# MarineRoboticsGroup/mac

Measured on AMD Instinct MI355X. Metric: frank_wolfe_iters_per_sec, higher is better.
Workload: dtype f64; 1 GPU; configs[3]: ER N=100000 ~2M candidates, chain fixed, K=10%; N=100000, m_candidates=2001737, K=200173, fixed_edges=99999, fw_iters=209, parallelism=single GPU

## Files before the change

### mac_amd/_lib.py

```python
from __future__ import annotations

import ctypes as C
import os

import numpy as np

_HERE = os.path.dirname(os.path.abspath(__file__))
LIB_PATH = os.environ.get("MACHIP_LIB") or os.path.join(_HERE, "libmachip.so")

OK, NOT_CONVERGED, DISCONNECTED, BAD_ARG, HIP_ERROR, RCCL_ERROR, NO_DEVICE = range(7)
STATUS_NAMES = ["OK", "NOT_CONVERGED", "DISCONNECTED", "BAD_ARG", "HIP_ERROR", "RCCL_ERROR", "NO_DEVICE"]


class MachipError(RuntimeError):
    def __init__(self, status, msg):
        super().__init__(f"libmachip: {STATUS_NAMES[status] if 0 <= status < 7 else status}: {msg}")
        self.status = status


class NotConverged(MachipError):
    pass


class Disconnected(MachipError):
# ... 68 lines not shown
    "machip_synchronize": (C.c_int, [C.c_void_p]),
    "machip_membench": (C.c_int, [C.c_int, C.c_int64, C.c_int, _f64p, _f64p]),
    "machip_host_tridiag_smallest": (C.c_int, [_f64p, _f64p, C.c_int, _f64p, _f64p]),
    "machip_host_follow_records": (C.c_int, [_f64p, C.c_int, C.c_int, C.c_double, C.c_double, C.c_int, C.POINTER(C.c_int), C.c_int,
                                             C.POINTER(C.c_int), C.POINTER(C.c_int), C.POINTER(C.c_double)]),
    "machip_release_cache": (None, []),
    "machip_panel_plan": (C.c_int, [C.c_int64, C.c_int64, C.c_int, C.POINTER(C.c_int)]),
    "machip_esp_create": (C.c_int, [C.c_int, C.c_int64, C.c_int64, _i32p, _i32p, _f64p, C.c_int64, _i32p, _i32p, _f64p,
                                    C.c_int, C.c_int, C.POINTER(C.c_void_p)]),
    "machip_esp_destroy": (None, [C.c_void_p]),
    "machip_esp_select": (C.c_int, [C.c_void_p, C.c_int, C.POINTER(C.c_int64), _i32p, _f64p, _f64p]),
    "machip_esp_weighted_resistances": (C.c_int, [C.c_void_p, _f64p]),
    "machip_esp_info": (C.c_int, [C.c_void_p, _i32p, C.POINTER(C.c_double)]),
    "machip_esp_tree_plan": (C.c_int, [C.c_int64, C.c_int64, _i32p, _i32p, _f64p, _i32p, _f64p, _i32p, _i32p, C.POINTER(C.c_int64),
                                       _i32p, _i32p, _f64p]),
    "machip_esp_seeds": (C.c_int, [C.c_void_p, C.POINTER(C.c_int64)]),
    "machip_esp_relax_eval": (C.c_int, [C.c_void_p, _f64p, C.POINTER(C.c_double), _f64p]),
    "machip_esp_relax_run": (C.c_int, [C.c_void_p, C.c_int64, C.c_int, C.c_double, C.c_double, _f64p, _f64p, _f64p, _f64p,
                                       C.POINTER(C.c_int), C.POINTER(C.c_double)]),
    "machip_esp_relax_inner": (C.c_int, [C.c_void_p, _f64p, _f64p, C.POINTER(C.c_double)]),
    "machip_esp_relax_info": (C.c_int, [C.c_void_p, _i32p]),
    "machip_esp_relax_gram": (C.c_int, [C.c_void_p, _f64p, C.c_int64]),
    "machip_esp_exchange": (C.c_int, [C.c_void_p, C.c_int64, _i32p, C.c_int64, C.c_double, _i32p, _i32p, _i32p, _f64p,
                                      C.POINTER(C.c_int64), C.POINTER(C.c_int32), _f64p]),
    "machip_eig_create": (C.c_int, [C.c_int, C.c_int64, C.c_int64, _i32p, _i32p, _f64p, C.c_int64, _i32p, _i32p, _f64p,
                                    C.c_int, C.c_int, C.c_int, C.POINTER(C.c_void_p)]),
    "machip_eig_destroy": (None, [C.c_void_p]),
    "machip_eig_select": (C.c_int, [C.c_void_p, C.c_int64, _i32p, _f64p, _f64p]),
    "machip_eig_candidate_lambda2": (C.c_int, [C.c_void_p, _f64p]),
    "machip_eig_candidate_bounds": (C.c_int, [C.c_void_p, _f64p]),
    "machip_eig_info": (C.c_int, [C.c_void_p, _i32p, _f64p, C.c_int64, _i32p, _i32p]),
}


def load():
    global _lib
    if _lib is not None:
        return _lib
    if not os.path.exists(LIB_PATH):
        raise ImportError(f"{LIB_PATH} is missing: build it with `python __graft_entry__.py` "
                          "(hipcc --offload-arch=gfx950); mac_amd has no CPU fallback")
    lib = C.CDLL(LIB_PATH, mode=C.RTLD_GLOBAL)
    for name, (res, args) in SIGNATURES.items():
        fn = getattr(lib, name)
        fn.restype = res
        fn.argtypes = args
    _lib = lib
    import atexit
    atexit.register(lib.machip_release_cache)
    return lib


OPTION_AUTO = -(1 << 63)
CREATION_OPTIONS = frozenset({"asm_g", "asm_maxgrid", "vbudget_mb", "vcap"})


def option_names():
    lib, out, i = load(), [], 0
    while True:
        nm = lib.machip_option_name(i)
        if nm is None:
            return out
        out.append(nm.decode())
        i += 1


def set_default_option(name, value=None):
    check(load().machip_set_option(None, name.encode(), OPTION_AUTO if value is None else int(value)))


class default_options:

    def __init__(self, **opts):
        self.opts = opts

    def __enter__(self):
        lib = load()
        self.old = {}
        for k, v in self.opts.items():
            cur = C.c_int64(0)
            check(lib.machip_get_option(None, k.encode(), C.byref(cur)))
            self.old[k] = cur.value
            set_default_option(k, v)
        return self

    def __exit__(self, *exc):
        for k, v in self.old.items():
            check(load().machip_set_option(None, k.encode(), v))
        return False


def membench(nbytes=1 << 30, reps=10, device=0):
    r, t = C.c_double(0.0), C.c_double(0.0)
    check(load().machip_membench(int(device), int(nbytes), int(reps), C.byref(r), C.byref(t)))
    return r.value, t.value


def device_count():
    return int(load().machip_device_count())


def require_device():
    n = device_count()
    if n <= 0:
        raise MachipError(NO_DEVICE, "no MI355X / HIP device visible; mac_amd has no CPU fallback")
    return n

# ... 512 lines not shown
```

### mac_amd/csrc/kernels.h

```cpp
#pragma once
#include "common.h"

namespace machip {

template <typename T>
struct CsrViewT {
    int n;
    const int* rowptr;
    const int* col;
    const T* val;
};
using CsrView = CsrViewT<double>;

struct PatternView {
    int n;
    const int* prow;
    const int* pcol;
    const int* pk;
    const double* pw;
};

struct LanState {
    int jA;
    int jB;
    int epoch;
    int jN;
};

struct LanView {
    int n;
    LanState* st;
    double* u;
    double* w;
    double* V;
    double* alpha;
    double* beta;
    double* l1;
    double* part_u;
    int P_u;
    double* part_a;
    int P_a;
};

constexpr int kAsmGrid = 4096;
__global__ __launch_bounds__(kBlock) void k_x_bits(const double* __restrict__ x, long m, double tol, unsigned long long* __restrict__ bits) {
    for (long i = (long)blockIdx.x * kBlock + threadIdx.x; i < m; i += (long)gridDim.x * kBlock) {
        const unsigned long long bal = __ballot(x[i] > tol);
        if ((threadIdx.x & 63) == 0) bits[i >> 6] = bal;
    }
}
__device__ __forceinline__ bool x_bit(const unsigned int* __restrict__ bits32, int k) { return (bits32[k >> 5] >> (k & 31)) & 1u; }

template <int G>
__global__ __launch_bounds__(kBlock) void k_asm_count(PatternView P, const unsigned int* __restrict__ xbits,
                                                      int rows_per_block,
                                                      int* __restrict__ cnt, int* __restrict__ blk_sum,
                                                      int* __restrict__ hsum = nullptr) {
    __shared__ int sm[4];
    constexpr int GPB = kBlock / G;
    const int lane = threadIdx.x % G, g = threadIdx.x / G;
    const int r0 = blockIdx.x * rows_per_block;
    const int r1 = min(P.n, r0 + rows_per_block);
    int local = 0, supp = 0, mx = 0;
    for (int r = r0 + g; r < r1; r += GPB) {
        const int b = P.prow[r], e = P.prow[r + 1];
        int c = 0, sc = 0;
        for (int p = b + lane; p < e; p += G) {
            const int k = P.pk[p];
            const bool cand = k >= 0;
            const bool act = cand ? x_bit(xbits, k) : true;
            c += act;
            sc += (cand && act);
        }
        c = group_sum_i<G>(c);
        sc = group_sum_i<G>(sc);
        if (lane == 0) {
            cnt[r] = c + 1;
            local += c + 1;
            supp += sc;
            mx = max(mx, c + 1);
        }
    }
    const int tot = block_sum_i(local, sm);
    const int stot = block_sum_i(supp, sm);
#pragma unroll
    for (int o = 32; o > 0; o >>= 1) mx = max(mx, __shfl_xor(mx, o, kWave));
    __syncthreads();
    if ((threadIdx.x & 63) == 0) sm[threadIdx.x >> 6] = mx;
    __syncthreads();
    if (threadIdx.x == 0) {
        blk_sum[blockIdx.x] = tot;
        blk_sum[kAsmGrid + blockIdx.x] = stot;
        const int longest = max(max(sm[0], sm[1]), max(sm[2], sm[3]));
        blk_sum[2 * kAsmGrid + blockIdx.x] = longest;
        if (hsum) {
            hsum[blockIdx.x] = tot; hsum[kAsmGrid + blockIdx.x] = stot; hsum[2 * kAsmGrid + blockIdx.x] = longest;
        }
    }
}

struct PanSpec {
    int NP = 0;
    int C = 1;
    int band = 0;
    int* ps = nullptr;
    double* bd = nullptr;
    int* bpk = nullptr;
    int* ovf = nullptr;
};

template <int G>
__global__ __launch_bounds__(kBlock) void k_asm_fill(PatternView P, const unsigned int* __restrict__ xbits, const double* __restrict__ x,
                                                     int rows_per_block,
                                                     const int* __restrict__ cnt,
                                                     const int* __restrict__ blk_sum,
                                                     int* __restrict__ rowptr, int* __restrict__ col,
                                                     double* __restrict__ val,
                                                     double* __restrict__ blk_lnorm, PanSpec S = PanSpec()) {
    extern __shared__ __attribute__((aligned(16))) char smem_raw[];
    int* s_off = reinterpret_cast<int*>(smem_raw);
    __shared__ int sm_i[4];
    __shared__ double sm_d[4];
    __shared__ int s_chunk[kBlock];
    constexpr int GPB = kBlock / G;
    const int tid = threadIdx.x;
    const int lane = tid % G, g = tid / G;
    const int r0 = blockIdx.x * rows_per_block;
    const int r1 = min(P.n, r0 + rows_per_block);
    const int nr = max(0, r1 - r0);

    int acc = 0;
    for (int b = tid; b < (int)blockIdx.x; b += kBlock) acc += blk_sum[b];
    const int base = block_sum_i(acc, sm_i);

    const int per = (nr + kBlock - 1) / kBlock;
    int csum = 0;
    for (int i = 0; i < per; ++i) {
        const int idx = tid * per + i;
        if (idx < nr) csum += cnt[r0 + idx];
    }
    {
        const int ln = tid & 63, wv = tid >> 6;
        int x = csum;
        for (int o = 1; o < 64; o <<= 1) { const int y = __shfl_up(x, o, kWave); if (ln >= o) x += y; }
        if (ln == 63) s_chunk[wv] = x;
        __syncthreads();
        int before = 0;
        for (int q = 0; q < wv; ++q) before += s_chunk[q];
        int run = before + x - csum;
        if (tid == kBlock - 1) s_off[nr] = before + x;
        for (int i = 0; i < per; ++i) {
            const int idx = tid * per + i;
            if (idx < nr) { s_off[idx] = run; run += cnt[r0 + idx]; }
        }
    }
    __syncthreads();

    double lmax = 0.0;
    for (int r = r0 + g; r < r1; r += GPB) {
        const int b = P.prow[r], e = P.prow[r + 1];
        const int out = base + s_off[r - r0];
        int pos = out + 1;
        double dsum = 0.0, asum = 0.0;
        int lastpid = 0;
        int hb = 0x7fffffff, hn = 0;
        double vl = 0.0, vu = 0.0;
        const int gbase = ((tid & 63) / G) * G;
        for (int p0 = b; p0 < e; p0 += G) {
            const int p = p0 + lane;
            const bool in = p < e;
            const int kc = in ? P.pk[p] : -1;
            const double wgt = in ? P.pw[p] : 0.0;
            const double xk = kc >= 0 ? x[kc] : 1.0;
            const bool act = in && (kc < 0 || x_bit(xbits, kc));
            const double v = act ? xk * wgt : 0.0;
            const unsigned long long bal = __ballot(act);
            unsigned long long gm;
            if (G == 64) gm = bal;
            else gm = (bal >> gbase) & ((1ull << (G & 63)) - 1ull);
            const unsigned long long below = gm & ((1ull << lane) - 1ull);
            const int before = __popcll(below);
            const int c = act ? P.pcol[p] : 0;
            if (act) { col[pos + before] = c; val[pos + before] = -v; }
            if (S.NP) {
                const int pid = act ? c / S.C : 0;
                const int src = below ? 63 - __builtin_clzll(below) : 0;
                const int got = __shfl(pid, gbase + src, kWave);
                const int ppid = below ? got : lastpid;
                if (act) {
                    const int q = pos + before;
                    for (int pp = ppid + 1; pp <= pid; ++pp) S.ps[(size_t)r * (S.NP + 1) + pp] = q;
                    if (S.band && (c == r - 1 || c == r + 1)) {
                        hb = min(hb, q); hn += 1;
                        if (c == r - 1) vl += -v; else vu += -v;
                    }
                }
                if (gm) lastpid = __shfl(pid, gbase + 63 - __builtin_clzll(gm), kWave);
            }
            pos += __popcll(gm);
            dsum += v;
            asum += fabs(v);
        }
        dsum = group_sum<G>(dsum);
        asum = group_sum<G>(asum);
        if (S.NP) {
            if (lane == 0) S.ps[(size_t)r * (S.NP + 1)] = out + 1;
            for (int pp = lastpid + 1 + lane; pp <= S.NP; pp += G) S.ps[(size_t)r * (S.NP + 1) + pp] = pos;
            if (S.band) {
                hn = group_sum_i<G>(hn);
                vl = group_sum<G>(vl); vu = group_sum<G>(vu);
#pragma unroll
                for (int o = G / 2; o > 0; o >>= 1) hb = min(hb, __shfl_xor(hb, o, kWave));
                if (lane == 0) {
                    S.bpk[r] = ((hn ? hb : pos) << 3) | min(hn, 7);
                    if (hn > 7) *S.ovf = 1;
                    S.bd[r] = dsum; S.bd[(size_t)P.n + r] = vl; S.bd[2 * (size_t)P.n + r] = vu;
                }
            }
        }
        if (lane == 0) {
            rowptr[r] = out;
            col[out] = r;
            val[out] = dsum;
            lmax = fmax(lmax, fabs(dsum) + asum);
        }
    }
    lmax = block_max(lmax, sm_d);
    if (tid == 0) {
        blk_lnorm[blockIdx.x] = lmax;
        if (blockIdx.x == gridDim.x - 1) rowptr[P.n] = base + s_off[nr];
    }
}

template <int G, class Op>
__device__ __forceinline__ void spmv_rows_vec(const CsrView& A, const double* __restrict__ x, Op& op) {
    constexpr int GPB = kBlock / G;
    const int lane = threadIdx.x % G, g = threadIdx.x / G;
    const int stride = gridDim.x * GPB;
    for (int r = blockIdx.x * GPB + g; r < A.n; r += 2 * stride) {
        const int r2 = r + stride;
        const bool two = r2 < A.n;
        const int b = A.rowptr[r], e = A.rowptr[r + 1];
        const int b2 = two ? A.rowptr[r2] : 0, e2 = two ? A.rowptr[r2 + 1] : 0;
        double acc = 0.0, acc2 = 0.0;
        int p = b + lane, q = b2 + lane;
        while (p < e || q < e2) {
            double v1 = 0.0, x1 = 0.0, v2 = 0.0, x2 = 0.0;
            if (p < e) { v1 = A.val[p]; x1 = op.gather(x, A.col[p]); }
            if (q < e2) { v2 = A.val[q]; x2 = op.gather(x, A.col[q]); }
            if (p < e) acc += v1 * x1;
            if (q < e2) acc2 += v2 * x2;
            p += G; q += G;
        }
        acc = group_sum<G>(acc);
        acc2 = group_sum<G>(acc2);
        if (lane == 0) { op.row(r, acc); if (two) op.row(r2, acc2); }
    }
}

constexpr int kStreamTile = 2048;

template <int TPR, class Op>
__device__ __forceinline__ void spmv_rows_stream(const CsrView& A, const double* __restrict__ x, Op& op,
                                                 double* prod, int* sptr) {
    constexpr int R = kBlock / TPR;
    const int tid = threadIdx.x;
    const int row = tid / TPR, sub = tid % TPR;
    for (int tile = blockIdx.x; tile * R < A.n; tile += gridDim.x) {
        const int r0 = tile * R;
        const int nr = min(R, A.n - r0);
        for (int i = tid; i <= nr; i += kBlock) sptr[i] = A.rowptr[r0 + i];
        __syncthreads();
        const int p0 = sptr[0], p1 = sptr[nr];
        double acc = 0.0;
        for (int base = p0; base < p1; base += kStreamTile) {
            const int cnt = min(kStreamTile, p1 - base);
            for (int i = tid; i < cnt; i += kBlock) prod[i] = A.val[base + i] * op.gather(x, A.col[base + i]);
            __syncthreads();
// ... 1130 lines not shown
```

### mac_amd/csrc/machip.hip

```cpp
#include <rccl/rccl.h>
#include <unistd.h>

#include <algorithm>
#include <atomic>
#include <cmath>
#include <chrono>
#include <condition_variable>
#include <functional>
#include <future>
#include <memory>
#include <mutex>
#include <numeric>
#include <thread>
#include <vector>

#include "solver.h"
#include "esp.h"
#include "esp_free.h"
#include "esp_tree.h"
#include "esp_relax.h"
#include "esp_exchange.h"
#include "eig.h"

namespace machip {
// ... 12 lines not shown
    auto state = std::make_shared<std::promise<int>>();
    std::future<int> fut = state->get_future();
    std::thread([state, fn] { int r = MACHIP_HIP_ERROR; try { r = fn(); } catch (...) {} state->set_value(r); }).detach();
    if (fut.wait_for(std::chrono::duration<double>(limit_s)) != std::future_status::ready)
        return fail(MACHIP_RCCL_ERROR, what + " did not return within " + std::to_string((int)limit_s) + " s (a peer rank is missing, or the fabric / bootstrap interface is not reachable; MACHIP_RCCL_TIMEOUT_S raises the limit)");
    return fut.get();
}
static double rccl_timeout_s() { const Options& opt = default_options(); const int t = OPT(rccl_timeout_s, 600); return t > 0 ? (double)t : 600.0; }

struct machip_problem;
struct LocalGroup {
    int nranks = 0;
    std::vector<double*> g;
    std::vector<machip_problem*> members;
    ShardGroup sg;
    bool shard_eig = false;
    int lead_status = MACHIP_OK;
    double lead_lam = 0.0;
    machip_solve_stats lead_stats{};
    std::string lead_err;
    ~LocalGroup() {
        for (ShardRank& r : sg.rk) for (hipEvent_t e : r.ev) if (e) (void)hipEventDestroy(e);
        if (sg.fork) (void)hipEventDestroy(sg.fork);
    }
    std::mutex mu;
    std::condition_variable cv;
    int waiting = 0;
    unsigned long generation = 0;
    bool broken = false;
    bool barrier() {
        std::unique_lock<std::mutex> lk(mu);
        if (broken) return false;
        const unsigned long gen = generation;
        if (++waiting == nranks) { waiting = 0; ++generation; cv.notify_all(); return true; }
        cv.wait(lk, [&] { return generation != gen || broken; });
        return !broken;
    }
    void abort() {
        std::lock_guard<std::mutex> lk(mu);
        broken = true;
        cv.notify_all();
    }
};

struct machip_problem {
    int device = 0;
    hipStream_t stream = nullptr;
    int n = 0;
    long m = 0, m_pad = 0;
    double tol_sel = 1e-10;
    int *prow = nullptr, *pcol = nullptr, *pk = nullptr;
    double* pw = nullptr;
    long P = 0;
    int asm_G = 16, asm_rpb = 1, asm_grid = 1;
    int *ci = nullptr, *cj = nullptr;
    double* cw = nullptr;
    double *x = nullptr, *x_next = nullptr, *g = nullptr, *s = nullptr, *scratch_m = nullptr;
    int *cnt = nullptr, *blk_sum = nullptr, *rowptr = nullptr, *col = nullptr;
    double *val = nullptr, *blk_lnorm = nullptr;
    unsigned long long *xb = nullptr, *xb_next = nullptr;
    bool xb_valid = false, xb_next_valid = false;
    long nnz = 0, support = 0;
    int maxlen = 0;
    double lnorm = 0.0;
    bool assembled = false, have_vec = false, csr_only = false;
    bool band_dups_ok = true;
    unsigned int* hist = nullptr;
    SelState* sel = nullptr;
    double* part_fw = nullptr;
    int* h_int = nullptr;
    double* h_dbl = nullptr;
    int* d_hint = nullptr;
    double* d_hdbl = nullptr;
    Solver sol;
    ncclComm_t comm = nullptr;
    std::shared_ptr<LocalGroup> lgroup;
    bool first_collective_pending = false;
    hipEvent_t ev_g0 = nullptr, ev_g1 = nullptr, ev_g2 = nullptr;
    bool ev_g_valid = false;
    std::unique_ptr<IpcGroup> ipcg;
    int rank = 0, nranks = 1;
    bool is_lane = false, lane_fw_ready = false;
    std::vector<machip_problem*> lanes;
    unsigned long start_version = 0;
    unsigned long seen_start_version = ~0ul;

    CsrView csr() const { return CsrView{n, rowptr, col, val}; }
    PatternView pattern() const { return PatternView{n, prow, pcol, pk, pw}; }
};

static int create_lane_stream(const Options& opt, int device, hipStream_t* out) {
    if (OPT(lane_queues, 0) == 0) {
        hipDeviceProp_t prop;
        if (hipGetDeviceProperties(&prop, device) == hipSuccess && prop.multiProcessorCount > 0) {
            const int words = (prop.multiProcessorCount + 31) / 32;
            std::vector<uint32_t> mask((size_t)words, 0xffffffffu);
            if (prop.multiProcessorCount % 32) mask.back() = (1u << (prop.multiProcessorCount % 32)) - 1u;
            if (hipExtStreamCreateWithCUMask(out, (uint32_t)words, mask.data()) == hipSuccess) return MACHIP_OK;
            (void)hipGetLastError();
        }
    }
    HIP_TRY(hipStreamCreateWithFlags(out, hipStreamNonBlocking));
    return MACHIP_OK;
}

namespace {

// ... 28 lines not shown
        const int a = fi[e], b = fj[e];
        if (a == b) continue;
        slots[(size_t)cur[(size_t)a]++] = Slot{b, -1, fw[e]};
        slots[(size_t)cur[(size_t)b]++] = Slot{a, -1, fw[e]};
    }
    for (int64_t e = 0; e < m; ++e) {
        const int a = ci[e], b = cj[e];
        if (a == b) continue;
        slots[(size_t)cur[(size_t)a]++] = Slot{b, (int)e, cw[e]};
        slots[(size_t)cur[(size_t)b]++] = Slot{a, (int)e, cw[e]};
    }
    std::vector<int> prow((size_t)n + 1, 0);
    std::vector<int> pcol, pk;
    std::vector<double> pw;
    pcol.reserve(slots.size()); pk.reserve(slots.size()); pw.reserve(slots.size());
    for (int r = 0; r < n; ++r) {
        Slot* b = slots.data() + off[(size_t)r];
        Slot* e = slots.data() + off[(size_t)r + 1];
        std::sort(b, e, [](const Slot& x, const Slot& y) {
            if (x.col != y.col) return x.col < y.col;
            return x.k < y.k;
        });
        for (Slot* q = b; q < e; ++q) {
            if (q->k < 0 && !pcol.empty() && (long)pcol.size() > prow[(size_t)r] && pcol.back() == q->col &&
                pk.back() < 0) {
                pw.back() += q->w;
            } else {
                pcol.push_back(q->col); pk.push_back(q->k); pw.push_back(q->w);
            }
        }
        if (pcol.size() > 2000000000ull) return fail(MACHIP_BAD_ARG, "pattern exceeds int32 indexing");
        {
            int band_slots = 0;
            for (size_t q = (size_t)prow[(size_t)r]; q < pcol.size(); ++q) band_slots += (pcol[q] == r - 1 || pcol[q] == r + 1);
            if (band_slots > 7) p->band_dups_ok = false;
        }
        prow[(size_t)r + 1] = (int)pcol.size();
    }
    p->P = (long)pcol.size();
    ST_TRY(dev_alloc(&p->prow, (size_t)n + 1));
    ST_TRY(dev_alloc(&p->pcol, (size_t)p->P)); ST_TRY(dev_alloc(&p->pk, (size_t)p->P)); ST_TRY(dev_alloc(&p->pw, (size_t)p->P));
    HIP_TRY(hipMemcpyAsync(p->prow, prow.data(), sizeof(int) * ((size_t)n + 1), hipMemcpyHostToDevice, p->stream));
    if (p->P) {
        HIP_TRY(hipMemcpyAsync(p->pcol, pcol.data(), sizeof(int) * (size_t)p->P, hipMemcpyHostToDevice, p->stream));
        HIP_TRY(hipMemcpyAsync(p->pk, pk.data(), sizeof(int) * (size_t)p->P, hipMemcpyHostToDevice, p->stream));
        HIP_TRY(hipMemcpyAsync(p->pw, pw.data(), sizeof(double) * (size_t)p->P, hipMemcpyHostToDevice, p->stream));
    }
    HIP_TRY(hipStreamSynchronize(p->stream));
    const double mean = n ? (double)p->P / n : 1.0;
    int G = 4;
    while (G < 64 && G < mean * 0.75) G <<= 1;
    p->asm_G = OPT(asm_g, G);
    const int gpb = kBlock / p->asm_G;
    long nblk = std::min<long>(std::min(kAsmGrid, std::max(1, OPT(asm_maxgrid, kAsmGrid))), ((long)n + gpb - 1) / gpb);
    if (nblk < 1) nblk = 1;
    long rpb = ((long)n + nblk - 1) / nblk;
    rpb = (rpb + gpb - 1) / gpb * gpb;
    p->asm_rpb = (int)rpb;
    p->asm_grid = (int)(((long)n + rpb - 1) / rpb);
    if (p->asm_grid < 1) p->asm_grid = 1;
    if ((rpb + 1) * (long)sizeof(int) > 64 * 1024)
        return fail(MACHIP_BAD_ARG, "num_nodes above the supported 16.7 million (row-offset scan of the assembly kernel)");
    return MACHIP_OK;
}

template <int G>
void launch_asm(machip_problem* p, const PanSpec& S) {
    const PatternView P = p->pattern();
    const unsigned int* xb32 = reinterpret_cast<const unsigned int*>(p->xb);
    k_asm_count<G><<<p->asm_grid, kBlock, 0, p->stream>>>(P, xb32, p->asm_rpb, p->cnt, p->blk_sum, p->d_hint);
    const size_t lds = sizeof(int) * ((size_t)p->asm_rpb + 1);
    k_asm_fill<G><<<p->asm_grid, kBlock, lds, p->stream>>>(P, xb32, p->x, p->asm_rpb, p->cnt, p->blk_sum,
                                                           p->rowptr, p->col, p->val, p->d_hdbl, S);
}

int assemble(machip_problem* p) {
    if (p->csr_only) return fail(MACHIP_BAD_ARG, "handle wraps a caller CSR; nothing to assemble");
    PanSpec S;
    ST_TRY(p->sol.pan_spec_prepare(&S));
    if (!p->xb_valid) {
        const int grid = std::max(1, (int)std::min<long>(kMaxGrid, (p->m + kBlock - 1) / kBlock));
        k_x_bits<<<grid, kBlock, 0, p->stream>>>(p->x, p->m, p->tol_sel, p->xb);
        p->xb_valid = true;
    }
    switch (p->asm_G) {
        case 4: launch_asm<4>(p, S); break;
        case 8: launch_asm<8>(p, S); break;
        case 16: launch_asm<16>(p, S); break;
        case 32: launch_asm<32>(p, S); break;
        default: launch_asm<64>(p, S); break;
    }
    HIP_TRY(hipGetLastError());
    const int gb = p->asm_grid;
    HIP_TRY(hipStreamSynchronize(p->stream));
    long nnz = 0, supp = 0;
    int maxlen = 0;
    double ln = 0.0;
    for (int b = 0; b < gb; ++b) {
        nnz += p->h_int[b]; supp += p->h_int[kAsmGrid + b]; maxlen = std::max(maxlen, p->h_int[2 * kAsmGrid + b]);
        ln = std::max(ln, p->h_dbl[b]);
    }
    p->nnz = nnz; p->support = supp / 2; p->lnorm = ln; p->maxlen = maxlen;
    p->assembled = true;
    return MACHIP_OK;
}

int alloc_common(machip_problem* p, int vbudget_mb = 0) {
    ST_TRY(p->sol.init(p->n, p->stream, vbudget_mb));
    HIP_TRY(hipHostMalloc((void**)&p->h_int, sizeof(int) * 3 * kAsmGrid, hipHostMallocMapped));
    HIP_TRY(hipHostMalloc((void**)&p->h_dbl, sizeof(double) * std::max(4 * kMaxGrid, kAsmGrid), hipHostMallocMapped));
    HIP_TRY(hipHostGetDevicePointer((void**)&p->d_hint, p->h_int, 0));
    HIP_TRY(hipHostGetDevicePointer((void**)&p->d_hdbl, p->h_dbl, 0));
    return MACHIP_OK;
}

int select_on(machip_problem* p, const double* keys, long k, SelState* st, int prefer_high, bool hist0_done = false) {
    const Options& opt = p->sol.opt;
    const long m = p->m;
    if (k < 0) k = 0;
    if (k > m) k = m;
    if (m <= kSelSmallMax && OPT(sel_small, 1)) {
        k_sel_small<<<1, 1024, 0, p->stream>>>(keys, m, (long long)k, st, prefer_high);
        HIP_TRY(hipGetLastError());
        return MACHIP_OK;
    }
    if (!hist0_done) k_sel_init<<<1, 1024, 0, p->stream>>>(st, (long long)k, p->hist, 6 * kBins);
// ... 775 lines not shown
    return run_with_watchdog([=]() -> int { std::this_thread::sleep_for(std::chrono::milliseconds(work_ms)); return MACHIP_OK; },
                             1e-3 * (double)limit_ms, "watchdog self-test (" + std::to_string(work_ms) + " ms of work)");
}

int machip_peer_access(int device_a, int device_b) {
    int can = 0;
    if (device_a == device_b) return 1;
    if (hipDeviceCanAccessPeer(&can, device_a, device_b) != hipSuccess) { (void)hipGetLastError(); return -1; }
    return can;
}

int machip_comm_mode(machip_problem* p) {
    if (!p) return -1;
    if (p->ipcg && p->ipcg->nranks) return p->sol.ipc ? (p->sol.last_seq_sharded ? 5 : 4) : (p->comm ? 1 : 6);
    if (p->comm) return 1;
    if (p->lgroup) return p->lgroup->shard_eig ? 3 : 2;
    return 0;
}

int machip_panel_plan(int64_t n, int64_t nnz, int maxlen, int* out12) {
    if (n < 1 || n > 2000000000ll || nnz < 0 || !out12) return fail(MACHIP_BAD_ARG, "machip_panel_plan: bad argument");
    const Options& opt = default_options();
    const PanPlan pp = plan_panel(opt, (int)n, (long)nnz, maxlen, true, -1, false, OPT(stream, 1) != 0);
    out12[0] = pp.on ? 1 : 0; out12[1] = pp.NP; out12[2] = pp.C; out12[3] = pp.NB; out12[4] = pp.NTB; out12[5] = pp.TWW; out12[6] = pp.RPT; out12[7] = pp.grid2;
    out12[8] = pp.u ? 1 : 0; out12[9] = pp.LPT; out12[10] = pp.TWT; out12[11] = pp.cells;
    return MACHIP_OK;
}

#ifdef PAN_CLOCKS
extern "C" int machip_debug_pan_clocks(machip_problem* p, long long* out, int groups) {
    if (!p || !out || groups < 1 || groups > kMaxGrid || !p->sol.panv.clk) return fail(MACHIP_BAD_ARG, "machip_debug_pan_clocks: no clock buffer");
    HIP_TRY(hipSetDevice(p->device));
    HIP_TRY(hipStreamSynchronize(p->stream));
    HIP_TRY(hipMemcpy(out, p->sol.panv.clk, sizeof(long long) * 16 * (size_t)groups, hipMemcpyDeviceToHost));
    HIP_TRY(hipMemset(p->sol.panv.clk, 0, sizeof(long long) * 16 * (size_t)kMaxGrid));
    return MACHIP_OK;
}
#endif

int machip_shard_plan(int64_t m, int nranks, int rank, int64_t* lo, int64_t* hi, int64_t* shard) {
    if (m < 0 || nranks < 1 || rank < 0 || rank >= nranks || !lo || !hi || !shard) return fail(MACHIP_BAD_ARG, "machip_shard_plan: bad argument");
    long a, b, c;
    shard_plan((long)m, nranks, rank, &a, &b, &c);
    *lo = a; *hi = b; *shard = c;
    return MACHIP_OK;
}

namespace {
int make_lane(machip_problem* p, machip_problem** out) {
    machip_problem* q = new machip_problem();
    q->is_lane = true;
    q->device = p->device; q->n = p->n; q->m = p->m; q->m_pad = p->m; q->tol_sel = p->tol_sel;
    q->prow = p->prow; q->pcol = p->pcol; q->pk = p->pk; q->pw = p->pw; q->P = p->P;
    q->asm_G = p->asm_G; q->asm_rpb = p->asm_rpb; q->asm_grid = p->asm_grid;
    q->ci = p->ci; q->cj = p->cj; q->cw = p->cw;
    auto body = [&]() -> int {
        ST_TRY(create_lane_stream(p->sol.opt, q->device, &q->stream));
        ST_TRY(dev_alloc(&q->x, (size_t)q->m + 64));
        const size_t cap = (size_t)q->P + (size_t)q->n + 8;
        ST_TRY(dev_alloc(&q->cnt, (size_t)q->n + 1)); ST_TRY(dev_alloc(&q->blk_sum, 3 * kAsmGrid));
        ST_TRY(dev_alloc(&q->rowptr, (size_t)q->n + 1)); ST_TRY(dev_alloc(&q->col, cap)); ST_TRY(dev_alloc(&q->val, cap));
        ST_TRY(dev_alloc(&q->blk_lnorm, kAsmGrid));
        ST_TRY(dev_alloc(&q->xb, (size_t)q->m / 64 + 2)); ST_TRY(dev_alloc(&q->xb_next, (size_t)q->m / 64 + 2));
        const Options& opt = p->sol.opt;
        q->sol.opt = opt;
        ST_TRY(alloc_common(q, std::max(16, OPT(lane_vbudget_mb, std::max(16, OPT(vbudget_mb, 4096) / 8)))));
        q->sol.csr_cap = cap;
        q->sol.pat = q->pattern();
        q->sol.pan_allowed = p->sol.pan_allowed;
        q->sol.chain_like = p->sol.chain_like; q->sol.chain_edges = p->sol.chain_edges;
        return MACHIP_OK;
    };
    const int st = body();
    if (st != MACHIP_OK) { machip_destroy(q); return st; }
    *out = q;
    return MACHIP_OK;
}

int ensure_lane_fw(machip_problem* q) {
    if (q->lane_fw_ready) return MACHIP_OK;
    const size_t mp = (size_t)q->m + 64 * 8;
    if (!q->x_next) ST_TRY(dev_alloc(&q->x_next, mp));
    if (!q->g) ST_TRY(dev_alloc(&q->g, mp));
    if (!q->s) ST_TRY(dev_alloc(&q->s, mp));
    if (!q->hist) ST_TRY(dev_alloc(&q->hist, (6 + kSelRep) * kBins));
    if (!q->sel) ST_TRY(dev_alloc(&q->sel, 2));
    if (!q->part_fw) ST_TRY(dev_alloc(&q->part_fw, 2 * kMaxGrid));
    HIP_TRY(hipMemsetAsync(q->g, 0, sizeof(double) * mp, q->stream));
    HIP_TRY(hipStreamSynchronize(q->stream));
    q->lane_fw_ready = true;
    return MACHIP_OK;
}

int prepare_lanes(machip_problem* p, int B, bool fw, int* nl_out) {
    const bool small = p->sol.chain_like && persist_fits(p->n, std::max(0l, (long)p->P - 2 * p->sol.chain_edges));
    const Options& opt = p->sol.opt;
    int nl = std::max(1, std::min(B, std::min(16, OPT(lanes, small ? 16 : 4))));
    while ((int)p->lanes.size() < nl) {
        machip_problem* q = nullptr;
        const int st = make_lane(p, &q);
        if (st != MACHIP_OK) {
            if (p->lanes.empty()) return st;
            (void)hipGetLastError();
            nl = (int)p->lanes.size();
            break;
        }
        p->lanes.push_back(q);
// ... 892 lines not shown
```

### mac_amd/csrc/options.h

```cpp
#pragma once
#include <climits>
#include <cstdlib>
#include <cstring>
#include <mutex>
#include <string>

namespace machip {

#define MACHIP_OPTION_LIST(X)                                                                                                      \
                                                                                                          \
    X(solver) X(graph) X(debug) X(chunk) X(chunk_near) X(sched) X(near_x10) X(trigger_pct) X(classic_n) X(persist) X(pchunk)      \
    X(spec_epilogue) X(spec_slack_pct) X(f32_switch_e9) X(tailless) X(stream) X(stream_trigger_pct) X(stream_retry_pct) X(stream_look) X(stream_margin) X(stream_window) X(stream_far) X(start_land) X(start_pow) X(start_floor_e6) X(start_land_pr_permille) X(start_land_min_mean10)                                                                \
                                                                        \
    X(spmv) X(g) X(unroll) X(block) X(maxgrid) X(defer) X(tpr) X(ell)                                                              \
                                                                                                            \
    X(panel) X(panel_min_n) X(panel_min_mean10) X(panel_multi_min_mean10) X(panel_np) X(panel_nb) X(panel_b2) X(panel_g2)         \
    X(panel_cells) X(panel_maxcells) X(panel_band) X(panel_u) X(panel_u_amp) X(pan32) X(pan32_switch_e9) X(panel_ops) X(panel_rev)                                                                               \
                                                                                                 \
    X(woodbury) X(wb_max) X(wb_hard) X(wb_lane_max) X(exact_big) X(exact_switch) X(gj_look_min) X(lob_density_pct) X(lob_chunk)   \
    X(lob_patience) X(lob_small_s) X(lob_fuse)                                                                                     \
     \
    X(sel_small) X(sel_fuse) X(asm_g) X(asm_maxgrid) X(vbudget_mb) X(vcap) X(lanes) X(lane_vbudget_mb) X(lane_queues) X(shard_eig) X(ipc_panel) \
    X(rccl_timeout_s)                                                                                                              \
               \
    X(esp_free_split)                                                                                                              \
       \
    X(esp_xch_lds_kb) X(esp_xch_max_mb) X(esp_xch_profile)

enum OptId {
#define X(n) kOpt_##n,
    MACHIP_OPTION_LIST(X)
#undef X
    kNumOpts
};

constexpr long kOptAuto = LONG_MIN;

inline const char* const* option_names() {
    static const char* const names[] = {
#define X(n) #n,
        MACHIP_OPTION_LIST(X)
#undef X
        nullptr};
    return names;
}
inline int option_id(const char* name) {
    if (!name) return -1;
    const char* const* nm = option_names();
    for (int i = 0; i < kNumOpts; ++i) if (!strcmp(nm[i], name)) return i;
    return -1;
}

struct Options {
    long v[kNumOpts];
    int get(OptId id, int dflt) const { return v[id] == kOptAuto ? dflt : (int)v[id]; }
    bool is_set(OptId id) const { return v[id] != kOptAuto; }
};

inline long option_parse(int id, const char* s) {
    if (id == kOpt_solver) {
        if (!strcmp(s, "auto")) return 0;
        if (!strcmp(s, "lanczos")) return 1;
        if (!strcmp(s, "lobpcg")) return 2;
    }
    if (id == kOpt_spmv) {
        if (!strcmp(s, "stream")) return 1;
        if (!strcmp(s, "vec")) return 2;
    }
    if (id == kOpt_lane_queues) {
        if (!strcmp(s, "shared")) return 1;
        if (!strcmp(s, "cumask")) return 0;
    }
    return atol(s);
}

// ... 20 lines not shown
```

Baseline: 133.9 iter/s.

## Batch row loads in Laplacian assembly kernels and shrink default assembly grid

Adds count and fill assembly kernels that process several rows per group at once. They issue the prow, pk, pw and pcol loads for the first slot chunks of each row up front, and in the fill kernel they prefetch the next batch while the current one is processed. This is meant to raise memory-level parallelism and hide gather latency in the per-iteration Laplacian assembly. The default assembly grid drops from 4096 to 2048 blocks, with rows per block rounded to a multiple of the batch factor. The cost is more register pressure, which may reduce occupancy.

After: 131.0 iter/s. 0.979x the previous value.

```diff
diff --git a/mac_amd/_lib.py b/mac_amd/_lib.py
--- a/mac_amd/_lib.py
+++ b/mac_amd/_lib.py
@@ -144,7 +144,7 @@
 
 
 OPTION_AUTO = -(1 << 63)
-CREATION_OPTIONS = frozenset({"asm_g", "asm_maxgrid", "vbudget_mb", "vcap"})
+CREATION_OPTIONS = frozenset({"asm_g", "asm_maxgrid", "asm_rf", "vbudget_mb", "vcap"})
 
 
 def option_names():
diff --git a/mac_amd/csrc/kernels.h b/mac_amd/csrc/kernels.h
--- a/mac_amd/csrc/kernels.h
+++ b/mac_amd/csrc/kernels.h
@@ -43,6 +43,7 @@
 };
 
 constexpr int kAsmGrid = 4096;
+constexpr int kAsmGridDflt = 2048;
 __global__ __launch_bounds__(kBlock) void k_x_bits(const double* __restrict__ x, long m, double tol, unsigned long long* __restrict__ bits) {
     for (long i = (long)blockIdx.x * kBlock + threadIdx.x; i < m; i += (long)gridDim.x * kBlock) {
         const unsigned long long bal = __ballot(x[i] > tol);
@@ -99,6 +100,84 @@
     }
 }
 
+constexpr int kAsmSB = 2;
+constexpr int kAsmRF = 2;
+template <int G, int RF>
+__global__ __launch_bounds__(kBlock) void k_asm_count_rf(PatternView P, int nslots, const unsigned int* __restrict__ xbits,
+                                                         int rows_per_block,
+                                                         int* __restrict__ cnt, int* __restrict__ blk_sum,
+                                                         int* __restrict__ hsum = nullptr) {
+    __shared__ int sm[4];
+    constexpr int GPB = kBlock / G, SB = kAsmSB;
+    const int lane = threadIdx.x % G, g = threadIdx.x / G;
+    const int r0 = blockIdx.x * rows_per_block;
+    const int r1 = min(P.n, r0 + rows_per_block);
+    int local = 0, supp = 0, mx = 0;
+    for (int rb = r0 + g; rb < r1; rb += GPB * RF) {
+        int b[RF], e[RF], k[RF][SB];
+        unsigned int w[RF][SB];
+#pragma unroll
+        for (int i = 0; i < RF; ++i) {
+            const int r = rb + i * GPB, rc = min(r, r1 - 1);
+            b[i] = P.prow[rc]; e[i] = P.prow[rc + 1];
+            if (r >= r1) e[i] = b[i];
+        }
+#pragma unroll
+        for (int i = 0; i < RF; ++i)
+#pragma unroll
+            for (int s = 0; s < SB; ++s) {
+                const int p = b[i] + s * G + lane;
+                k[i][s] = P.pk[p < e[i] ? p : min(b[i], nslots - 1)];
+            }
+#pragma unroll
+        for (int i = 0; i < RF; ++i)
+#pragma unroll
+            for (int s = 0; s < SB; ++s) w[i][s] = xbits[max(k[i][s], 0) >> 5];
+#pragma unroll
+        for (int i = 0; i < RF; ++i) {
+            const int r = rb + i * GPB;
+            int c = 0, sc = 0;
+#pragma unroll
+            for (int s = 0; s < SB; ++s) {
+                const bool in = b[i] + s * G + lane < e[i];
+                const bool cand = k[i][s] >= 0;
+                const bool act = in && (cand ? (w[i][s] >> (k[i][s] & 31)) & 1u : true);
+                c += act;
+                sc += (cand && act);
+            }
+            for (int p = b[i] + SB * G + lane; p < e[i]; p += G) {
+                const int kk = P.pk[p];
+                const bool cand = kk >= 0;
+                const bool act = cand ? x_bit(xbits, kk) : true;
+                c += act;
+                sc += (cand && act);
+            }
+            c = group_sum_i<G>(c);
+            sc = group_sum_i<G>(sc);
+            if (lane == 0 && r < r1) {
+                cnt[r] = c + 1;
+                local += c + 1;
+                supp += sc;
+                mx = max(mx, c + 1);
+            }
+        }
+    }
+    const int tot = block_sum_i(local, sm);
+    const int stot = block_sum_i(supp, sm);
+#pragma unroll
+    for (int o = 32; o > 0; o >>= 1) mx = max(mx, __shfl_xor(mx, o, kWave));
+    __syncthreads();
+    if ((threadIdx.x & 63) == 0) sm[threadIdx.x >> 6] = mx;
+    __syncthreads();
+    if (threadIdx.x == 0) {
+        blk_sum[blockIdx.x] = tot;
+        blk_sum[kAsmGrid + blockIdx.x] = stot;
+        const int longest = max(max(sm[0], sm[1]), max(sm[2], sm[3]));
+        blk_sum[2 * kAsmGrid + blockIdx.x] = longest;
+        if (hsum) { hsum[blockIdx.x] = tot; hsum[kAsmGrid + blockIdx.x] = stot; hsum[2 * kAsmGrid + blockIdx.x] = longest; }
+    }
+}
+
 struct PanSpec {
     int NP = 0;
     int C = 1;
@@ -108,6 +187,107 @@
     int* bpk = nullptr;
     int* ovf = nullptr;
 };
+
+struct AsmRow {
+    int pos;
+    double dsum = 0.0, asum = 0.0;
+    int lastpid = 0;
+    int hb = 0x7fffffff, hn = 0;
+    double vl = 0.0, vu = 0.0;
+};
+
+template <int G>
+__device__ __forceinline__ void asm_slots(AsmRow& R, int r, int lane, int gbase, bool live, bool act, double v, int c,
+                                          int* __restrict__ col, double* __restrict__ val, const PanSpec& S) {
+    const unsigned long long bal = __ballot(act);
+    unsigned long long gm;
+    if (G == 64) gm = bal;
+    else gm = (bal >> gbase) & ((1ull << (G & 63)) - 1ull);
+    const unsigned long long below = gm & ((1ull << lane) - 1ull);
+    const int before = __popcll(below);
+    if (act) { col[R.pos + before] = c; val[R.pos + before] = -v; }
+    if (S.NP) {
+        const int pid = act ? c / S.C : 0;
+        const int src = below ? 63 - __builtin_clzll(below) : 0;
+        const int got = __shfl(pid, gbase + src, kWave);
+        const int ppid = below ? got : R.lastpid;
+        if (act) {
+            const int q = R.pos + before;
+            for (int pp = ppid + 1; pp <= pid; ++pp) S.ps[(size_t)r * (S.NP + 1) + pp] = q;
+            if (S.band && (c == r - 1 || c == r + 1)) {
+                R.hb = min(R.hb, q); R.hn += 1;
+                if (c == r - 1) R.vl += -v; else R.vu += -v;
+            }
+        }
+        if (gm) R.lastpid = __shfl(pid, gbase + 63 - __builtin_clzll(gm), kWave);
+    }
+    R.pos += __popcll(gm);
+    if (live) { R.dsum += v; R.asum += fabs(v); }
+}
+
+template <int G>
+__device__ __forceinline__ double asm_row_end(AsmRow& R, int r, int n, int out, int lane, bool has,
+                                              int* __restrict__ rowptr, int* __restrict__ col, double* __restrict__ val,
+                                              const PanSpec& S) {
+    const double dsum = group_sum<G>(R.dsum);
+    const double asum = group_sum<G>(R.asum);
+    if (S.NP) {
+        if (lane == 0 && has) S.ps[(size_t)r * (S.NP + 1)] = out + 1;
+        if (has)
+            for (int pp = R.lastpid + 1 + lane; pp <= S.NP; pp += G) S.ps[(size_t)r * (S.NP + 1) + pp] = R.pos;
+        if (S.band) {
+            const int hn = group_sum_i<G>(R.hn);
+            const double vl = group_sum<G>(R.vl), vu = group_sum<G>(R.vu);
+            int hb = R.hb;
+#pragma unroll
+            for (int o = G / 2; o > 0; o >>= 1) hb = min(hb, __shfl_xor(hb, o, kWave));
+            if (lane == 0 && has) {
+                S.bpk[r] = ((hn ? hb : R.pos) << 3) | min(hn, 7);
+                if (hn > 7) *S.ovf = 1;
+                S.bd[r] = dsum; S.bd[(size_t)n + r] = vl; S.bd[2 * (size_t)n + r] = vu;
+            }
+        }
+    }
+    if (lane == 0 && has) {
+        rowptr[r] = out;
+        col[out] = r;
+        val[out] = dsum;
+        return fabs(dsum) + asum;
+    }
+    return 0.0;
+}
+
+__device__ __forceinline__ int asm_fill_head(const int* __restrict__ cnt, const int* __restrict__ blk_sum, int r0, int nr,
+                                             int* s_off, int* sm_i, int* s_chunk) {
+    const int tid = threadIdx.x;
+    int acc = 0;
+    for (int b = tid; b < (int)blockIdx.x; b += kBlock) acc += blk_sum[b];
+    const int base = block_sum_i(acc, sm_i);
+
+    const int per = (nr + kBlock - 1) / kBlock;
+    int csum = 0;
+    for (int i = 0; i < per; ++i) {
+        const int idx = tid * per + i;
+        if (idx < nr) csum += cnt[r0 + idx];
+    }
+    {
+        const int ln = tid & 63, wv = tid >> 6;
+        int x = csum;
+        for (int o = 1; o < 64; o <<= 1) { const int y = __shfl_up(x, o, kWave); if (ln >= o) x += y; }
+        if (ln == 63) s_chunk[wv] = x;
+        __syncthreads();
+        int before = 0;
+        for (int q = 0; q < wv; ++q) before += s_chunk[q];
+        int run = before + x - csum;
+        if (tid == kBlock - 1) s_off[nr] = before + x;
+        for (int i = 0; i < per; ++i) {
+            const int idx = tid * per + i;
+            if (idx < nr) { s_off[idx] = run; run += cnt[r0 + idx]; }
+        }
+    }
+    __syncthreads();
+    return base;
+}
 
 template <int G>
 __global__ __launch_bounds__(kBlock) void k_asm_fill(PatternView P, const unsigned int* __restrict__ xbits, const double* __restrict__ x,
@@ -129,43 +309,15 @@
     const int r1 = min(P.n, r0 + rows_per_block);
     const int nr = max(0, r1 - r0);
 
-    int acc = 0;
-    for (int b = tid; b < (int)blockIdx.x; b += kBlock) acc += blk_sum[b];
-    const int base = block_sum_i(acc, sm_i);
-
-    const int per = (nr + kBlock - 1) / kBlock;
-    int csum = 0;
-    for (int i = 0; i < per; ++i) {
-        const int idx = tid * per + i;
-        if (idx < nr) csum += cnt[r0 + idx];
-    }
-    {
-        const int ln = tid & 63, wv = tid >> 6;
-        int x = csum;
-        for (int o = 1; o < 64; o <<= 1) { const int y = __shfl_up(x, o, kWave); if (ln >= o) x += y; }
-        if (ln == 63) s_chunk[wv] = x;
-        __syncthreads();
-        int before = 0;
-        for (int q = 0; q < wv; ++q) before += s_chunk[q];
-        int run = before + x - csum;
-        if (tid == kBlock - 1) s_off[nr] = before + x;
-        for (int i = 0; i < per; ++i) {
-            const int idx = tid * per + i;
-            if (idx < nr) { s_off[idx] = run; run += cnt[r0 + idx]; }
-        }
-    }
-    __syncthreads();
+    const int base = asm_fill_head(cnt, blk_sum, r0, nr, s_off, sm_i, s_chunk);
 
     double lmax = 0.0;
+    const int gbase = ((tid & 63) / G) * G;
     for (int r = r0 + g; r < r1; r += GPB) {
         const int b = P.prow[r], e = P.prow[r + 1];
         const int out = base + s_off[r - r0];
-        int pos = out + 1;
-        double dsum = 0.0, asum = 0.0;
-        int lastpid = 0;
-        int hb = 0x7fffffff, hn = 0;
-        double vl = 0.0, vu = 0.0;
-        const int gbase = ((tid & 63) / G) * G;
+        AsmRow R;
+        R.pos = out + 1;
         for (int p0 = b; p0 < e; p0 += G) {
             const int p = p0 + lane;
             const bool in = p < e;
@@ -174,56 +326,114 @@
             const double xk = kc >= 0 ? x[kc] : 1.0;
             const bool act = in && (kc < 0 || x_bit(xbits, kc));
             const double v = act ? xk * wgt : 0.0;
-            const unsigned long long bal = __ballot(act);
-            unsigned long long gm;
-            if (G == 64) gm = bal;
-            else gm = (bal >> gbase) & ((1ull << (G & 63)) - 1ull);
-            const unsigned long long below = gm & ((1ull << lane) - 1ull);
-            const int before = __popcll(below);
             const int c = act ? P.pcol[p] : 0;
-            if (act) { col[pos + before] = c; val[pos + before] = -v; }
-            if (S.NP) {
-                const int pid = act ? c / S.C : 0;
-                const int src = below ? 63 - __builtin_clzll(below) : 0;
-                const int got = __shfl(pid, gbase + src, kWave);
-                const int ppid = below ? got : lastpid;
-                if (act) {
-                    const int q = pos + before;
-                    for (int pp = ppid + 1; pp <= pid; ++pp) S.ps[(size_t)r * (S.NP + 1) + pp] = q;
-                    if (S.band && (c == r - 1 || c == r + 1)) {
-                        hb = min(hb, q); hn += 1;
-                        if (c == r - 1) vl += -v; else vu += -v;
-                    }
-                }
-                if (gm) lastpid = __shfl(pid, gbase + 63 - __builtin_clzll(gm), kWave);
-            }
-            pos += __popcll(gm);
-            dsum += v;
-            asum += fabs(v);
-        }
-        dsum = group_sum<G>(dsum);
-        asum = group_sum<G>(asum);
-        if (S.NP) {
-            if (lane == 0) S.ps[(size_t)r * (S.NP + 1)] = out + 1;
-            for (int pp = lastpid + 1 + lane; pp <= S.NP; pp += G) S.ps[(size_t)r * (S.NP + 1) + pp] = pos;
-            if (S.band) {
-                hn = group_sum_i<G>(hn);
-                vl = group_sum<G>(vl); vu = group_sum<G>(vu);
-#pragma unroll
-                for (int o = G / 2; o > 0; o >>= 1) hb = min(hb, __shfl_xor(hb, o, kWave));
-                if (lane == 0) {
-                    S.bpk[r] = ((hn ? hb : pos) << 3) | min(hn, 7);
-                    if (hn > 7) *S.ovf = 1;
-                    S.bd[r] = dsum; S.bd[(size_t)P.n + r] = vl; S.bd[2 * (size_t)P.n + r] = vu;
-                }
-            }
-        }
-        if (lane == 0) {
-            rowptr[r] = out;
-            col[out] = r;
-            val[out] = dsum;
-            lmax = fmax(lmax, fabs(dsum) + asum);
-        }
+            asm_slots<G>(R, r, lane, gbase, true, act, v, c, col, val, S);
+        }
+        lmax = fmax(lmax, asm_row_end<G>(R, r, P.n, out, lane, true, rowptr, col, val, S));
+    }
+    lmax = block_max(lmax, sm_d);
+    if (tid == 0) {
+        blk_lnorm[blockIdx.x] = lmax;
+        if (blockIdx.x == gridDim.x - 1) rowptr[P.n] = base + s_off[nr];
+    }
+}
+
+template <int G, int RF>
+__global__ __launch_bounds__(kBlock) void k_asm_fill_rf(PatternView P, int nslots, const unsigned int* __restrict__ xbits,
+                                                        const double* __restrict__ x, int rows_per_block,
+                                                        const int* __restrict__ cnt, const int* __restrict__ blk_sum,
+                                                        int* __restrict__ rowptr, int* __restrict__ col, double* __restrict__ val,
+                                                        double* __restrict__ blk_lnorm, PanSpec S = PanSpec()) {
+    extern __shared__ __attribute__((aligned(16))) char smem_raw[];
+    int* s_off = reinterpret_cast<int*>(smem_raw);
+    __shared__ int sm_i[4];
+    __shared__ double sm_d[4];
+    __shared__ int s_chunk[kBlock];
+    constexpr int GPB = kBlock / G, SB = kAsmSB, GPW = kWave / G;
+    const int tid = threadIdx.x;
+    const int lane = tid % G, g = tid / G;
+    const int r0 = blockIdx.x * rows_per_block;
+    const int r1 = min(P.n, r0 + rows_per_block);
+    const int nr = max(0, r1 - r0);
+    const int gf = (tid >> 6) * GPW;
+    const int nrow_f = r0 + gf < r1 ? (r1 - r0 - gf + GPB - 1) / GPB : 0;
+    const int nbat = __builtin_amdgcn_readfirstlane((nrow_f + RF - 1) / RF);
+
+    int b[RF], e[RF], k[RF][SB], c[RF][SB];
+    double w[RF][SB];
+    auto load_batch = [&](int t) {
+#pragma unroll
+        for (int i = 0; i < RF; ++i) {
+            const int r = r0 + g + (t * RF + i) * GPB, rc = min(r, r1 - 1);
+            b[i] = P.prow[rc]; e[i] = P.prow[rc + 1];
+            if (r >= r1) e[i] = b[i];
+        }
+#pragma unroll
+        for (int i = 0; i < RF; ++i)
+#pragma unroll
+            for (int s = 0; s < SB; ++s) {
+                const int p = b[i] + s * G + lane;
+                const int q = p < e[i] ? p : min(b[i], nslots - 1);
+                k[i][s] = P.pk[q]; w[i][s] = P.pw[q]; c[i][s] = P.pcol[q];
+            }
+    };
+    load_batch(0);
+
+    const int base = asm_fill_head(cnt, blk_sum, r0, nr, s_off, sm_i, s_chunk);
+
+    double lmax = 0.0;
+    const int gbase = ((tid & 63) / G) * G;
+    for (int t = 0; t < nbat; ++t) {
+        double xk[RF][SB];
+        unsigned int bw[RF][SB];
+#pragma unroll
+        for (int i = 0; i < RF; ++i)
+#pragma unroll
+            for (int s = 0; s < SB; ++s) {
+                const int kk = max(k[i][s], 0);
+                xk[i][s] = x[kk]; bw[i][s] = xbits[kk >> 5];
+            }
+        double v[RF][SB];
+        unsigned int am = 0;
+#pragma unroll
+        for (int i = 0; i < RF; ++i)
+#pragma unroll
+            for (int s = 0; s < SB; ++s) {
+                const bool in = b[i] + s * G + lane < e[i];
+                const bool act = in && (k[i][s] < 0 || ((bw[i][s] >> (k[i][s] & 31)) & 1u));
+                const double xv = k[i][s] >= 0 ? xk[i][s] : 1.0;
+                v[i][s] = act ? xv * w[i][s] : 0.0;
+                am |= (unsigned int)act << (i * SB + s);
+            }
+#pragma unroll
+        for (int i = 0; i < RF; ++i) {
+            const int r = r0 + g + (t * RF + i) * GPB;
+            const bool has = r < r1;
+            if (__ballot(has) == 0ull) break;
+            const int out = base + s_off[has ? r - r0 : 0];
+            AsmRow R;
+            R.pos = out + 1;
+#pragma unroll
+            for (int s = 0; s < SB; ++s) {
+                const int p0 = b[i] + s * G;
+                if (__ballot(p0 + lane < e[i]) == 0ull) continue;
+                const bool act = (am >> (i * SB + s)) & 1u;
+                asm_slots<G>(R, r, lane, gbase, p0 < e[i], act, v[i][s], act ? c[i][s] : 0, col, val, S);
+            }
+            for (int p0 = b[i] + SB * G; __ballot(p0 < e[i]) != 0ull; p0 += G) {
+                const int p = p0 + lane;
+                const bool in = p < e[i];
+                const int kt = in ? P.pk[p] : -1;
+                const double wt = in ? P.pw[p] : 0.0;
+                const int ct = in ? P.pcol[p] : 0;
+                const double xt = kt >= 0 ? x[kt] : 1.0;
+                const bool act = in && (kt < 0 || x_bit(xbits, kt));
+                const double v = act ? xt * wt : 0.0;
+                asm_slots<G>(R, r, lane, gbase, p0 < e[i], act, v, act ? ct : 0, col, val, S);
+            }
+            lmax = fmax(lmax, asm_row_end<G>(R, r, P.n, out, lane, has, rowptr, col, val, S));
+        }
+        if (t + 1 < nbat) load_batch(t + 1);
     }
     lmax = block_max(lmax, sm_d);
     if (tid == 0) {
diff --git a/mac_amd/csrc/machip.hip b/mac_amd/csrc/machip.hip
--- a/mac_amd/csrc/machip.hip
+++ b/mac_amd/csrc/machip.hip
@@ -88,7 +88,7 @@
     int *prow = nullptr, *pcol = nullptr, *pk = nullptr;
     double* pw = nullptr;
     long P = 0;
-    int asm_G = 16, asm_rpb = 1, asm_grid = 1;
+    int asm_G = 16, asm_rpb = 1, asm_grid = 1, asm_rf = 0;
     int *ci = nullptr, *cj = nullptr;
     double* cw = nullptr;
     double *x = nullptr, *x_next = nullptr, *g = nullptr, *s = nullptr, *scratch_m = nullptr;
@@ -223,10 +223,13 @@
     while (G < 64 && G < mean * 0.75) G <<= 1;
     p->asm_G = OPT(asm_g, G);
     const int gpb = kBlock / p->asm_G;
-    long nblk = std::min<long>(std::min(kAsmGrid, std::max(1, OPT(asm_maxgrid, kAsmGrid))), ((long)n + gpb - 1) / gpb);
+    long nblk = std::min<long>(std::min(kAsmGrid, std::max(1, OPT(asm_maxgrid, kAsmGridDflt))), ((long)n + gpb - 1) / gpb);
     if (nblk < 1) nblk = 1;
     long rpb = ((long)n + nblk - 1) / nblk;
     rpb = (rpb + gpb - 1) / gpb * gpb;
+    const int rf_opt = OPT(asm_rf, kAsmRF);
+    p->asm_rf = p->P == 0 ? 0 : rf_opt >= 8 ? 8 : rf_opt >= 4 ? 4 : rf_opt >= 2 ? 2 : 0;
+    if (p->asm_rf && rpb / gpb >= p->asm_rf) rpb = (rpb + (long)gpb * p->asm_rf - 1) / ((long)gpb * p->asm_rf) * ((long)gpb * p->asm_rf);
     p->asm_rpb = (int)rpb;
     p->asm_grid = (int)(((long)n + rpb - 1) / rpb);
     if (p->asm_grid < 1) p->asm_grid = 1;
@@ -235,14 +238,29 @@
     return MACHIP_OK;
 }
 
-template <int G>
+template <int G, int RF>
 void launch_asm(machip_problem* p, const PanSpec& S) {
     const PatternView P = p->pattern();
     const unsigned int* xb32 = reinterpret_cast<const unsigned int*>(p->xb);
-    k_asm_count<G><<<p->asm_grid, kBlock, 0, p->stream>>>(P, xb32, p->asm_rpb, p->cnt, p->blk_sum, p->d_hint);
     const size_t lds = sizeof(int) * ((size_t)p->asm_rpb + 1);
-    k_asm_fill<G><<<p->asm_grid, kBlock, lds, p->stream>>>(P, xb32, p->x, p->asm_rpb, p->cnt, p->blk_sum,
-                                                           p->rowptr, p->col, p->val, p->d_hdbl, S);
+    if constexpr (RF == 0) {
+        k_asm_count<G><<<p->asm_grid, kBlock, 0, p->stream>>>(P, xb32, p->asm_rpb, p->cnt, p->blk_sum, p->d_hint);
+        k_asm_fill<G><<<p->asm_grid, kBlock, lds, p->stream>>>(P, xb32, p->x, p->asm_rpb, p->cnt, p->blk_sum,
+                                                               p->rowptr, p->col, p->val, p->d_hdbl, S);
+    } else {
+        k_asm_count_rf<G, RF><<<p->asm_grid, kBlock, 0, p->stream>>>(P, (int)p->P, xb32, p->asm_rpb, p->cnt, p->blk_sum, p->d_hint);
+        k_asm_fill_rf<G, RF><<<p->asm_grid, kBlock, lds, p->stream>>>(P, (int)p->P, xb32, p->x, p->asm_rpb, p->cnt, p->blk_sum,
+                                                                      p->rowptr, p->col, p->val, p->d_hdbl, S);
+    }
+}
+template <int G>
+void launch_asm(machip_problem* p, const PanSpec& S) {
+    switch (p->asm_rf) {
+        case 2: launch_asm<G, 2>(p, S); break;
+        case 4: launch_asm<G, 4>(p, S); break;
+        case 8: launch_asm<G, 8>(p, S); break;
+        default: launch_asm<G, 0>(p, S); break;
+    }
 }
 
 int assemble(machip_problem* p) {
@@ -1124,7 +1142,7 @@
     q->is_lane = true;
     q->device = p->device; q->n = p->n; q->m = p->m; q->m_pad = p->m; q->tol_sel = p->tol_sel;
     q->prow = p->prow; q->pcol = p->pcol; q->pk = p->pk; q->pw = p->pw; q->P = p->P;
-    q->asm_G = p->asm_G; q->asm_rpb = p->asm_rpb; q->asm_grid = p->asm_grid;
+    q->asm_G = p->asm_G; q->asm_rpb = p->asm_rpb; q->asm_grid = p->asm_grid; q->asm_rf = p->asm_rf;
     q->ci = p->ci; q->cj = p->cj; q->cw = p->cw;
     auto body = [&]() -> int {
         ST_TRY(create_lane_stream(p->sol.opt, q->device, &q->stream));
diff --git a/mac_amd/csrc/options.h b/mac_amd/csrc/options.h
--- a/mac_amd/csrc/options.h
+++ b/mac_amd/csrc/options.h
@@ -20,7 +20,7 @@
     X(woodbury) X(wb_max) X(wb_hard) X(wb_lane_max) X(exact_big) X(exact_switch) X(gj_look_min) X(lob_density_pct) X(lob_chunk)   \
     X(lob_patience) X(lob_small_s) X(lob_fuse)                                                                                     \
      \
-    X(sel_small) X(sel_fuse) X(asm_g) X(asm_maxgrid) X(vbudget_mb) X(vcap) X(lanes) X(lane_vbudget_mb) X(lane_queues) X(shard_eig) X(ipc_panel) \
+    X(sel_small) X(sel_fuse) X(asm_g) X(asm_maxgrid) X(asm_rf) X(vbudget_mb) X(vcap) X(lanes) X(lane_vbudget_mb) X(lane_queues) X(shard_eig) X(ipc_panel) \
     X(rccl_timeout_s)                                                                                                              \
                \
     X(esp_free_split)                                                                                                              \
```
